# koszullab/chromosight

Measured on AMD Instinct MI355X. Metric: Mpixels/s normxcorr2 (17x17 loops kernel), higher is better.
Workload: dtype f32

## Files before the change

chromosight_amd/csrc/cs_corr_mfma.hip:

```cpp
#include "cs_device.h"
#include <algorithm>
#include <cstdlib>
#include <cstring>
#include <mutex>
#include <utility>
#include <vector>

#include "cs_launch.h"

namespace cs {

typedef _Float16 h8 __attribute__((ext_vector_type(8)));

__device__ __forceinline__ float cand_range_guard(float r, float s2, float unscale, const KernelStats<float>& K);
typedef _Float16 h4 __attribute__((ext_vector_type(4)));
typedef float f4 __attribute__((ext_vector_type(4)));
typedef float f4u __attribute__((ext_vector_type(4), aligned(4)));
typedef double d2u __attribute__((ext_vector_type(2), aligned(8)));

constexpr int MF_T = 64;
constexpr int MF_R = 80;
constexpr int MF_PLANE = MF_R * MF_R * 2;
constexpr int MF_WSET = 17 * 2 * 1024;
constexpr int MF_SCR_PITCH = 40;
constexpr int MF_SCR_PLANE = 16 * MF_SCR_PITCH * 2;
constexpr int MF_SMEM = 3 * MF_PLANE + MF_WSET + 64;
constexpr int MF_PER_THREAD = (MF_R * MF_R) / 256;

static_assert(5 * MF_SCR_PLANE * 4 <= MF_WSET, "scratch aliases the weight region");

#ifdef CS_MF_DEBUG
#define MFD_DBG(bit) (A.dbg & (bit))
#else
#define MFD_DBG(bit) (false)
#endif

#ifdef CS_MF_PROFILE
__device__ unsigned long long cs_mf_prof[16];
#define MF_STAMP(k)                                                        \
    do {                                                                   \
        const unsigned long long now_ = __builtin_readcyclecounter();      \
        if (tid == 0) MF_PROF_ADD(k, now_ - tprev_);                       \
        tprev_ = now_;                                                     \
    } while (0)
#define MF_PROF_ADD(k, v) atomicAdd(&cs_mf_prof[k], (unsigned long long)(v))
#else
#define MF_STAMP(k)
#endif

__device__ __forceinline__ f4 mfma16(const h8& a, const h8& b, const f4& c)
{
    return __builtin_amdgcn_mfma_f32_16x16x32_f16(a, b, c, 0, 0, 0);
}

template <bool MASKED>
__global__ __launch_bounds__(256, 2) void corr_mfma_kernel(const CorrArgs<float> A, const MfmaWeights E)
{
    extern __shared__ __attribute__((aligned(16))) char smem[];
    _Float16* xh = reinterpret_cast<_Float16*>(smem);
    _Float16* xl = reinterpret_cast<_Float16*>(smem + MF_PLANE);
    _Float16* xm = reinterpret_cast<_Float16*>(smem + 2 * MF_PLANE);
    char* wreg = smem + 3 * MF_PLANE;
    unsigned* red = reinterpret_cast<unsigned*>(wreg + MF_WSET);

    const int tid = threadIdx.x;
    const int lane = tid & 63, wv = tid >> 6;
    const int n = lane & 15, g = lane >> 4;

    const int by = blockIdx.x / A.tiles_x;
    const int bx = blockIdx.x - by * A.tiles_x;
    const int I0 = A.row_begin + by * MF_T;
    if (I0 >= A.row_end) return;
    const bool band_out = A.out.layout == 1;
    const int J0 = band_out ? I0 + A.out_lo + bx * MF_T : bx * MF_T;
    if (J0 >= A.ns || J0 + MF_T <= 0) return;
    if (J0 + MF_T - 1 - I0 < A.out_lo || J0 - (I0 + MF_T - 1) > A.out_hi) return;
#ifdef CS_MF_PROFILE
    unsigned long long tprev_ = __builtin_readcyclecounter();
    if (tid == 0) atomicAdd(&cs_mf_prof[15], 1ull);
#endif
    const int km = A.km, kn = A.kn;
    const int P0 = I0 - (km - 1) / 2, Q0 = J0 - (kn - 1) / 2;
    const int p_lo = A.row_begin - (km - 1) / 2, p_hi = A.row_end + (km - 1) - (km - 1) / 2;

    float xv[MF_PER_THREAD];
    unsigned miss_bits = 0, ok_bits = 0;
    long long offs[MF_PER_THREAD];
#pragma unroll
    for (int k = 0; k < MF_PER_THREAD; ++k) {
        const int idx = tid + 256 * k;
        const int r = idx / MF_R, c = idx - r * MF_R;
        const int p = P0 + r, q = Q0 + c;
        const bool inside = (p >= 0) & (p < A.ms) & (q >= 0) & (q < A.ns) & (p >= p_lo) & (p < p_hi);
        const long long off = inside ? mat_offset(A.sig, p, q) : -1;
        if (off >= 0) ok_bits |= 1u << k;
        offs[k] = off >= 0 ? off : 0;
    }
    if (A.sig_is_f64) {
        const double* src = reinterpret_cast<const double*>(A.sig.ptr);
#pragma unroll
        for (int k = 0; k < MF_PER_THREAD; ++k) xv[k] = (float)src[offs[k]];
    } else {
        const float* src = reinterpret_cast<const float*>(A.sig.ptr);
#pragma unroll
        for (int k = 0; k < MF_PER_THREAD; ++k) xv[k] = src[offs[k]];
    }
    if constexpr (MASKED) {
        unsigned char fr[MF_PER_THREAD], fc[MF_PER_THREAD];
        if (A.mask_mode == 1) {
#pragma unroll
            for (int k = 0; k < MF_PER_THREAD; ++k) {
                const int idx = tid + 256 * k;
                const int r = idx / MF_R, c = idx - r * MF_R;
                fr[k] = A.miss_row[min(max(P0 + r, 0), A.ms - 1)];
                fc[k] = A.miss_col[min(max(Q0 + c, 0), A.ns - 1)];
            }
        } else {
            const unsigned char* mp = reinterpret_cast<const unsigned char*>(A.mask.ptr);
#pragma unroll
            for (int k = 0; k < MF_PER_THREAD; ++k) {
                fr[k] = mp[offs[k]];
                fc[k] = 0;
            }
        }
#pragma unroll
        for (int k = 0; k < MF_PER_THREAD; ++k) {
            const int idx = tid + 256 * k;
            const int r = idx / MF_R, c = idx - r * MF_R;
            const int p = P0 + r, q = Q0 + c;
            const bool stored = (ok_bits >> k) & 1u;
            const bool needed = (p >= p_lo) & (p < p_hi);
            if (needed && missing_from_flags(A, p, q, fr[k] != 0, fc[k] != 0, fr[k] != 0, stored)) miss_bits |= 1u << k;
        }
    }
    float amax = 0.0f;
#pragma unroll
    for (int k = 0; k < MF_PER_THREAD; ++k) {
        const float x = (((ok_bits & ~miss_bits) >> k) & 1u) ? xv[k] : 0.0f;
        xv[k] = x;
        amax = fmaxf(amax, fabsf(x));
    }
    MF_STAMP(0);
    if (tid == 0) *red = 0u;
    __syncthreads();
#pragma unroll
    for (int off = 32; off >= 1; off >>= 1) amax = fmaxf(amax, __shfl_xor(amax, off));
    if (lane == 0) atomicMax(red, __float_as_uint(amax));
    __syncthreads();
    int ex = 0;
    {
        const int e = (int)((*red >> 23) & 0xffu);
        if (e != 0 && e != 255) ex = 6 - (e - 127);
        ex = max(-100, min(100, ex));
    }
    const float scale = __uint_as_float((unsigned)(ex + 127) << 23);
    const float unscale = __uint_as_float((unsigned)(127 - ex) << 23);
#pragma unroll
    for (int k = 0; k < MF_PER_THREAD; ++k) {
        const int idx = tid + 256 * k;
        const float xs = xv[k] * scale;
        const _Float16 h = (_Float16)xs;
        xh[idx] = h;
        xl[idx] = (_Float16)(xs - (float)h);
        if constexpr (MASKED) xm[idx] = (miss_bits >> k) & 1u ? (_Float16)1.0f : (_Float16)0.0f;
    }
    __syncthreads();

    MF_STAMP(1);
    h8 ones_b, ones_a;
#pragma unroll
    for (int e = 0; e < 8; ++e) {
        const int t = 8 * g + e - n;
        ones_b[e] = (t >= 0 && t < kn) ? (_Float16)1.0f : (_Float16)0.0f;
        ones_a[e] = (t >= 0 && t < km) ? (_Float16)1.0f : (_Float16)0.0f;
    }
    const f4 zero4 = {0.0f, 0.0f, 0.0f, 0.0f};
    const int wr0 = 16 * wv;

    f4 S1[4], S2[4], NM[4];
    char* scr = wreg + wv * (5 * MF_SCR_PLANE);
#pragma unroll
    for (int c = 0; c < 4; ++c) {
#pragma unroll
        for (int rb = 0; rb < 2; ++rb) {
            const int off = (wr0 + 16 * rb + n) * MF_R + 16 * c + 8 * g;
            const h8 ah = *reinterpret_cast<const h8*>(xh + off);
            const h8 al = *reinterpret_cast<const h8*>(xl + off);
            f4 h1 = mfma16(ah, ones_b, zero4);
            h1 = mfma16(al, ones_b, h1);
            h8 qh, ql;
#pragma unroll
            for (int e = 0; e < 8; ++e) {
                const float x = (float)ah[e] + (float)al[e];
                const float q = x * x * 0.03125f;
                qh[e] = (_Float16)q;
                ql[e] = (_Float16)(q - (float)qh[e]);
            }
            f4 h2 = mfma16(qh, ones_b, zero4);
            h2 = mfma16(ql, ones_b, h2);
            h4 t1h, t1l, t2h, t2l;
#pragma unroll
            for (int v = 0; v < 4; ++v) {
                t1h[v] = (_Float16)h1[v];
                t1l[v] = (_Float16)(h1[v] - (float)t1h[v]);
                t2h[v] = (_Float16)h2[v];
                t2l[v] = (_Float16)(h2[v] - (float)t2h[v]);
            }
            const int so = (n * MF_SCR_PITCH + 16 * rb + 4 * g) * 2;
            *reinterpret_cast<h4*>(scr + 0 * MF_SCR_PLANE + so) = t1h;
            *reinterpret_cast<h4*>(scr + 1 * MF_SCR_PLANE + so) = t1l;
            *reinterpret_cast<h4*>(scr + 2 * MF_SCR_PLANE + so) = t2h;
            *reinterpret_cast<h4*>(scr + 3 * MF_SCR_PLANE + so) = t2l;
            if constexpr (MASKED) {
                const h8 am = *reinterpret_cast<const h8*>(xm + off);
                const f4 hm = mfma16(am, ones_b, zero4);
                h4 tm;
#pragma unroll
                for (int v = 0; v < 4; ++v) tm[v] = (_Float16)hm[v];
                *reinterpret_cast<h4*>(scr + 4 * MF_SCR_PLANE + so) = tm;
            }
        }
        __syncthreads();
        {
            const int ro = (n * MF_SCR_PITCH + 8 * g) * 2;
            const h8 b1h = *reinterpret_cast<const h8*>(scr + 0 * MF_SCR_PLANE + ro);
            const h8 b1l = *reinterpret_cast<const h8*>(scr + 1 * MF_SCR_PLANE + ro);
            const h8 b2h = *reinterpret_cast<const h8*>(scr + 2 * MF_SCR_PLANE + ro);
            const h8 b2l = *reinterpret_cast<const h8*>(scr + 3 * MF_SCR_PLANE + ro);
            S1[c] = mfma16(ones_a, b1h, zero4);
            S1[c] = mfma16(ones_a, b1l, S1[c]);
            S2[c] = mfma16(ones_a, b2h, zero4);
            S2[c] = mfma16(ones_a, b2l, S2[c]);
            NM[c] = zero4;
            if constexpr (MASKED) {
                const h8 bm = *reinterpret_cast<const h8*>(scr + 4 * MF_SCR_PLANE + ro);
                NM[c] = mfma16(ones_a, bm, zero4);
            }
        }
        __syncthreads();
    }

    MF_STAMP(2);
    auto load_set = [&](int set) {
        const uint4* src = E.frag + (size_t)set * km * 128;
        uint4* dst = reinterpret_cast<uint4*>(wreg);
        for (int idx = tid; idx < km * 128; idx += 256) dst[idx] = src[idx];
    };
    f4 accM[4], accC[4], KA[4], KB[4];
#pragma unroll
    for (int c = 0; c < 4; ++c) accM[c] = accC[c] = KA[c] = KB[c] = zero4;

    load_set(0);
    __syncthreads();
    MF_STAMP(3);
    for (int s = 0; s < km; ++s) {
        const h8 bh = reinterpret_cast<const h8*>(wreg)[(2 * s + 0) * 64 + lane];
        const h8 bl = reinterpret_cast<const h8*>(wreg)[(2 * s + 1) * 64 + lane];
#pragma unroll
        for (int c = 0; c < 4; ++c) {
            const int off = (wr0 + s + n) * MF_R + 16 * c + 8 * g;
            const h8 ah = *reinterpret_cast<const h8*>(xh + off);
            const h8 al = *reinterpret_cast<const h8*>(xl + off);
            accM[c] = mfma16(ah, bh, accM[c]);
            accC[c] = mfma16(ah, bl, accC[c]);
            accC[c] = mfma16(al, bh, accC[c]);
        }
    }
    MF_STAMP(4);
    if constexpr (MASKED) {
        for (int set = 1; set <= 2; ++set) {
            __syncthreads();
            load_set(set);
            __syncthreads();
            for (int s = 0; s < km; ++s) {
                const h8 bh = reinterpret_cast<const h8*>(wreg)[(2 * s + 0) * 64 + lane];
                const h8 bl = reinterpret_cast<const h8*>(wreg)[(2 * s + 1) * 64 + lane];
#pragma unroll
                for (int c = 0; c < 4; ++c) {
                    const int off = (wr0 + s + n) * MF_R + 16 * c + 8 * g;
                    const h8 am = *reinterpret_cast<const h8*>(xm + off);
                    if (set == 1) {
                        KA[c] = mfma16(am, bh, KA[c]);
                        KA[c] = mfma16(am, bl, KA[c]);
                    } else {
                        KB[c] = mfma16(am, bh, KB[c]);
                        KB[c] = mfma16(am, bl, KB[c]);
                    }
                }
            }
        }
    }

    MF_STAMP(5);
    const float u_cs = unscale * E.unscale[0];
    const float u_s2 = 32.0f * unscale;
#pragma unroll
    for (int c = 0; c < 4; ++c) {
        const int j = J0 + 16 * c + n;
#pragma unroll
        for (int v = 0; v < 4; ++v) {
            const int i = I0 + wr0 + 4 * g + v;
            if (i >= A.row_end || j < 0 || j >= A.ns) continue;
            const int d = j - i;
            if (d < A.out_lo || d > A.out_hi) continue;
            const float cs = (accM[c][v] + accC[c][v]) * u_cs;
            const float s1 = S1[c][v] * unscale;
            const float s2 = (S2[c][v] * u_s2) * unscale;
            float r, nobs = A.ks.n;
            if (pixel_forced_zero(A, i, j)) {
                r = 0.0f;
            } else if (A.xcorr_only) {
                r = (fabsf(cs) < A.ks.thr) ? 0.0f : cs;
            } else if constexpr (MASKED) {
                const float nm = NM[c][v];
                const float ka = KA[c][v] * E.unscale[1], kb = KB[c][v] * E.unscale[2];
                r = cand_range_guard(pearson_masked_lean(cs, s1, s2, nm, ka, kb, A.ks), s2, unscale, A.ks);
                nobs = A.ks.n - nm;
            } else {
                r = cand_range_guard(pearson_nomask_lean(cs, s1, s2, A.ks), s2, unscale, A.ks);
            }
            store_pixel(A, i, j, r, nobs);
        }
    }
    MF_STAMP(6);
}

#ifdef CS_MF_PROFILE
extern "C" int cs_debug_mfma_profile(unsigned long long* out)
{
    hipError_t e = hipMemcpyFromSymbol(out, HIP_SYMBOL(cs_mf_prof), sizeof(cs_mf_prof));
    if (e != hipSuccess) return (int)e;
    unsigned long long zero[16] = {0};
    return (int)hipMemcpyToSymbol(HIP_SYMBOL(cs_mf_prof), zero, sizeof(zero));
}
#endif

struct MfmaFixArgs {
    int fix_on, fix_hi_w, fix_hi_d0;
    const float* fix_lo;
    const float* fix_hi;
    const float* fix_rows;
    const float* fix_cols;
    int fix_top, fix_bot0, fix_width, fix_xband, fix_xlo, fix_side;
    const float* rim;
    int max_dist;
};

struct MfmaDenseArgs {
    const float* sig;
    void* out;
    int out_is_f64;
    long long ld_in, ld_out, row0_in, row0_out;
    int ms, ns, km, kn;
    int row_begin, row_end;
    int full, sym_upper;
    int xcorr_only;
    int tiles_x, n_tiles;
    int by_cut;
    const uint4* frag;
    float w_unscale;
    float wa_unscale, wb_unscale;
    int xcd_order;
    int dbg;
    KernelStats<float> ks;
    int band_in, lo_in, bw_in;
    int pad_in;
    int cnt_in;
    int band_out, lo_out;
    int out_lo, out_hi;
    float* nobs;
    const float* w;
    const uint8_t* miss_col;
    const float* rowtab;
    const float* coltab;
    int fix_on, fix_hi_w, fix_hi_d0, fix_top, fix_bot0, fix_any_side;
    int rim_in_kernel;
    MfmaFixArgs fx;
};

constexpr int MFD_ROWS_PER_THREAD = 14;
constexpr int MFD_WL = 4 * MF_PLANE;
constexpr int MFD_SCR = MFD_WL + 18 * 1024;
constexpr int MFD_RED = MFD_SCR + 4 * 2 * MF_SCR_PLANE;
constexpr int MFD_SMEM = MFD_RED + 64;
constexpr int MFD_COL = MFD_RED + 64;
constexpr int MFD_CFL = MFD_COL + 2 * 3 * 64 * 4;
constexpr int MFD_CFB = MFD_CFL + 2 * 16;
constexpr int MFD_SMEM_REG = MFD_CFB + 2 * 128;
static_assert(MFD_SMEM_REG <= 80 * 1024, "two workgroups per CU");
#ifdef CS_MF_PROFILE
constexpr int MFD_PROF = MFD_SMEM_REG;
constexpr int MFD_LAUNCH_EXTRA = 128;
#else
constexpr int MFD_LAUNCH_EXTRA = 0;
#endif

__device__ __forceinline__ unsigned pack_h2(_Float16 a, _Float16 b)
{
    typedef _Float16 h2 __attribute__((ext_vector_type(2)));
    h2 v;
    v[0] = a;
    v[1] = b;
    return __builtin_bit_cast(unsigned, v);
}

__device__ __forceinline__ float sub_f16_lo(float x, unsigned h)
{
    float r;
    asm("v_fma_mix_f32 %0, -%1, 1.0, %2 op_sel_hi:[1,0,0]" : "=v"(r) : "v"(h), "v"(x));
    return r;
}

__device__ __forceinline__ float sub_f16_hi(float x, unsigned h)
{
    float r;
    asm("v_fma_mix_f32 %0, -%1, 1.0, %2 op_sel:[1,0,0] op_sel_hi:[1,0,0]" : "=v"(r) : "v"(h), "v"(x));
    return r;
}

__device__ __forceinline__ void lds_barrier()
{
    __builtin_amdgcn_fence(__ATOMIC_RELEASE, "workgroup", "local");
    __builtin_amdgcn_s_waitcnt(0xc07f);
    __builtin_amdgcn_s_barrier();
    __builtin_amdgcn_fence(__ATOMIC_ACQUIRE, "workgroup", "local");
}

__device__ __forceinline__ float wave_max_nonneg(float v)
{
#define CS_DPP_MAX(ctrl, rmask)                                                                                  \
    v = fmaxf(v, __builtin_bit_cast(float, __builtin_amdgcn_update_dpp(0, __builtin_bit_cast(int, v), ctrl, rmask, 0xf, true)))
    CS_DPP_MAX(0x111, 0xf);
    CS_DPP_MAX(0x112, 0xf);
    CS_DPP_MAX(0x114, 0xf);
    CS_DPP_MAX(0x118, 0xf);
    CS_DPP_MAX(0x142, 0xa);
    CS_DPP_MAX(0x143, 0xc);
#undef CS_DPP_MAX
    return v;
}

__device__ __forceinline__ void wave_lds_sync()
{
    __builtin_amdgcn_fence(__ATOMIC_RELEASE, "wavefront");
    __builtin_amdgcn_wave_barrier();
    __builtin_amdgcn_fence(__ATOMIC_ACQUIRE, "wavefront");
}

__device__ __forceinline__ float cand_range_guard(float r, float s2, float unscale, const KernelStats<float>& K)
{
    if (K.cand_cmin > 0.0f) r = ((int)(s2 > 0.0f) & (int)(s2 < K.n * (unscale * unscale) * 0.0625f)) ? 2.0f : r;
    return r;
}

__device__ __attribute__((noinline)) float masked_coefficient_rare(float cs, float s1, float s2, float nm, float ka, float kb,
                                                                   const KernelStats<float>& K)
{
    return pearson_masked_f32(cs, s1, s2, nm, ka, kb, K);
}

__device__ __forceinline__ float masked_coefficient(float cs, float s1, float s2, float nm, float ka, float kb,
                                                    const KernelStats<float>& K)
{
    bool rare;
    float r = pearson_masked_core(cs, s1, s2, nm, ka, kb, K, rare);
    if (rare) r = masked_coefficient_rare(cs, s1, s2, nm, ka, kb, K);
    return r;
}

typedef const __attribute__((address_space(4))) MfmaFixArgs* FixArgsPtr;

__device__ __forceinline__ FixArgsPtr fix_args()
{
    unsigned long long kv = (unsigned long long)__builtin_amdgcn_kernarg_segment_ptr();
    asm volatile("" : "+s"(kv));
    return (FixArgsPtr)(kv + offsetof(MfmaDenseArgs, fx));
}

typedef const __attribute__((address_space(4))) KernelStats<float>* StatsPtr;

__device__ __forceinline__ StatsPtr stats_args()
{
    unsigned long long kv = (unsigned long long)__builtin_amdgcn_kernarg_segment_ptr();
    asm volatile("" : "+s"(kv));
    return (StatsPtr)(kv + offsetof(MfmaDenseArgs, ks));
}
// ... 459 lines not shown
```

chromosight_amd/csrc/cs_corr_mfma_body.inc:

```

    extern __shared__ __attribute__((aligned(16))) char smem[];
    char* const pl_xh = smem;
    char* const pl_xl = smem + MF_PLANE;
    char* const pl_qh = smem + 2 * MF_PLANE;
    char* const pl_ql = smem + 3 * MF_PLANE;
    float* const raw = reinterpret_cast<float*>(smem + 2 * MF_PLANE);
    const int tid = threadIdx.x;
    const int lane = tid & 63, wv = tid >> 6;
    const int n = lane & 15, g = lane >> 4;
    char* const scr = smem + MFD_SCR + wv * (2 * MF_SCR_PLANE);
    unsigned* const red = reinterpret_cast<unsigned*>(smem + MFD_RED);
    const int km = A.km, kn = A.kn;
    const int kh = (km - 1) / 2, kw = (kn - 1) / 2;
#ifdef CS_MF_PROFILE
#undef MF_PROF_ADD
#define MF_PROF_ADD(k, v) (prof_lds[k] += (unsigned long long)(v))
    unsigned long long* const prof_lds = reinterpret_cast<unsigned long long*>(smem + MFD_PROF);
    unsigned long long tprev_ = 0;
    if (tid == 0)
        for (int k = 0; k < 16; ++k) prof_lds[k] = 0;
    auto prof_flush = [&]() {
        if (tid == 0)
            for (int k = 0; k < 16; ++k)
                if (prof_lds[k]) atomicAdd(&cs_mf_prof[k], prof_lds[k]);
    };
#endif

    h8 ones_b, ones_p;
#pragma unroll
    for (int e = 0; e < 8; ++e) {
        const int t = 8 * g + e - n;
        ones_b[e] = (t >= 0 && t < kn) ? (_Float16)1.0f : (_Float16)0.0f;
        const int rho = (e < 4 ? 4 * g + e : 16 + 4 * g + (e - 4)) - n;
        ones_p[e] = (rho >= 0 && rho < km) ? (_Float16)1.0f : (_Float16)0.0f;
    }
    const f4 zero4 = {0.0f, 0.0f, 0.0f, 0.0f};
    const int wr0 = 16 * wv;
    const int c2 = tid % 40, rg = tid / 40;
    const int c2_ = c2, rg_ = rg;
    const bool stager = tid < 240;
    const int p_min = max(0, A.row_begin - kh), p_max = min(A.ms, A.row_end + (km - 1) - kh) - 1;
    int pad_row0 = 0x7fffffff;
    if constexpr (REG && VEC4) pad_row0 = A.pad_in ? max(p_min, (int)A.row0_in + 1) : 0x7fffffff;
    float cnt_max = 0.0f;
    const float* cnt_wt = nullptr;
    const float* cnt_rlaw = nullptr;
    int cnt_n = 1, cnt_nd = 1;
    if constexpr (REG && VEC4) {
        if (A.cnt_in) {
            const CountsHdrPtr H = counts_header(A.sig);
            cnt_max = (float)H->max_val;
            cnt_wt = H->weight32;
            cnt_rlaw = H->rlaw32;
            cnt_n = H->n;
            cnt_nd = H->n_diags;
        }
    }

    auto tile_origin = [&](int tile, int& I0, int& J0) {
        if constexpr (LIST) tile = tile_list[tile];
        int by = tile / A.tiles_x;
        int bx = tile - by * A.tiles_x;
        if constexpr (REG) {
            if (by >= A.by_cut) {
                int t = tile - A.by_cut * A.tiles_x;
                by = A.by_cut;
                for (;;) {
                    const int left = A.ns - (A.row_begin + by * MF_T + A.out_lo);
                    const int v = min(A.tiles_x, left <= 0 ? 0 : (left + MF_T - 1) / MF_T);
                    if (t < v) break;
                    t -= v;
                    ++by;
                }
                bx = t;
            }
        }
        I0 = A.row_begin + by * MF_T;
        if constexpr (!REG) {
            const int skew = A.xcd_order >> 1;
            if (skew) {
                bx += (by * skew) % A.tiles_x;
                bx -= bx >= A.tiles_x ? A.tiles_x : 0;
            }
        }
        J0 = bx * MF_T;
        if (REG && A.band_out) J0 += I0 + A.out_lo;
    };
    const int wv_u = __builtin_amdgcn_readfirstlane(wv);
    auto fetch_args = [&]() {
        if constexpr (REG) return TABLE ? args_at(table_entry) : args_here();
        else return &A;
    };
    constexpr int kPiecesPerRow = VEC4 ? MF_R / 4 : MF_R;
    constexpr int kTransfers = VEC4 ? 25 : 100;
    auto fetch = [&](int tile, int slot) {
        const auto FA = fetch_args();
        int I0, J0;
        tile_origin(tile, I0, J0);
        const int P0 = I0 - kh, Q0 = J0 - kw;
        const bool pad_tile = REG && VEC4 && P0 >= pad_row0 && P0 + MF_R - 1 <= p_max;
        int lane_f = lane;
        if constexpr (REG) asm volatile("" : "+v"(lane_f));
        const int e0 = 64 * wv_u + lane_f;
        int r = e0 / kPiecesPerRow, c = e0 - r * kPiecesPerRow;
        if (REG && !MFD_DBG(16384)) {
            if (wv_u < 3) {
                const float* src = FA->coltab + (size_t)wv_u * FA->ns + min(max(J0 + lane_f, 0), FA->ns - 1);
                __builtin_amdgcn_global_load_lds(src, (__attribute__((address_space(3))) void*)(
                    (__attribute__((address_space(3))) char*)(smem) + MFD_COL + (slot * 3 + wv_u) * 256), 4, 0, 0);
            } else {
                const long long base = (long long)(uintptr_t)FA->miss_col;
                const long long first = ((base + Q0) >> 2) << 2;
                long long addr = first + 4 * min(lane_f, 23);
                addr = min(max(addr, (base >> 2) << 2), ((base + FA->ns - 1) >> 2) << 2);
                if (lane_f < 24)
                    __builtin_amdgcn_global_load_lds(reinterpret_cast<const unsigned*>((uintptr_t)addr),
                                                     (__attribute__((address_space(3))) void*)(
                                                         (__attribute__((address_space(3))) char*)(smem) + MFD_CFB + slot * 128), 4, 0, 0);
            }
        }
        if constexpr (REG && VEC4) {
            if (FA->cnt_in) {
                const float* wt = cnt_wt;
                const float* rlaw = cnt_rlaw;
                const int hn = cnt_n, hd = cnt_nd;
#pragma unroll 1
                for (int x = wv_u; x < 5; x += 4) {
                    const int e = 64 * x + lane_f;
                    const bool is_w = e < 160;
                    const int idx = e < 80 ? P0 + e : e < 160 ? Q0 + (e - 80) : Q0 - P0 - (MF_R - 1) + (e - 160);
                    const float* src = (is_w ? wt : rlaw) + min(max(idx, is_w ? 0 : -1), is_w ? hn - 1 : hd);
                    __builtin_amdgcn_global_load_lds(src, (__attribute__((address_space(3))) void*)(
                                                              (__attribute__((address_space(3))) char*)(smem) + MFD_SCR + 256 * x), 4, 0, 0);
                }
            }
        }
        const __attribute__((address_space(3))) char* dst =
            (const __attribute__((address_space(3))) char*)(raw) + (VEC4 ? 1024 : 256) * wv_u;
        if constexpr (!REG && VEC4) {
            if (P0 >= p_min && P0 + MF_R - 1 <= p_max && Q0 >= 0 && Q0 + MF_R <= FA->ns) {
                const float* src = FA->sig + ((long long)P0 + r - FA->row0_in) * FA->ld_in + Q0 + 4 * c;
                const long long step_r = 12 * FA->ld_in + 64, wrap = FA->ld_in - 80;
#pragma unroll 1
                for (int i = wv_u; i < kTransfers; i += 4) {
                    __builtin_amdgcn_global_load_lds(src, (__attribute__((address_space(3))) void*)dst, 16, 0, 0);
                    dst += 4096;
                    c += 16;
                    src += step_r;
                    if (c >= kPiecesPerRow) {
                        c -= kPiecesPerRow;
                        src += wrap;
                    }
                }
                return;
            }
        }
        if constexpr (REG && VEC4) {
            if (FA->band_in && P0 >= p_min && P0 + MF_R - 1 <= p_max && Q0 - (P0 + MF_R - 1) - FA->lo_in >= 0 &&
                Q0 + MF_R - 1 - P0 - FA->lo_in <= FA->bw_in - 1) {
                const float* src = FA->sig + ((long long)P0 - FA->row0_in) * FA->ld_in + (Q0 - P0 - FA->lo_in) + (long long)r * (FA->ld_in - 1) + 4 * c;
                const long long step_r = 12 * (FA->ld_in - 1) + 64, wrap = (FA->ld_in - 1) - 80;
#pragma unroll 1
                for (int i = wv_u; i < kTransfers; i += 4) {
                    __builtin_amdgcn_global_load_lds(src, (__attribute__((address_space(3))) void*)dst, 16, 0, 0);
                    dst += 4096;
                    c += 16;
                    src += step_r;
                    if (c >= kPiecesPerRow) {
                        c -= kPiecesPerRow;
                        src += wrap;
                    }
// ... 396 lines not shown
                           (!A.sym_upper || J0 - (I0 + MF_T - 1) + (A.full ? kn - km : 0) >= 0);
        const int i = I0 + wr0 + n;
        const long long o_idx = ((long long)i - A.row0_out) * A.ld_out + (J0 + 4 * g);
        f4 rv[4];
        bool lean = !A.xcorr_only && !MFD_DBG(32) && !(MFD_NOMASK_KS.cand_cmin > 0.0f);
        if (lean) {
            const KernelStats<float>& KS = MFD_NOMASK_KS;
            const float inv_u = __uint_as_float((254u << 23) - __float_as_uint(unscale));
            const float t1 = KS.thr_n * inv_u;
            const float t2 = (t1 * inv_u) * 0.03125f;
            const float td = (KS.den2_min * inv_u) * inv_u;
            const float top = (fmaxf(KS.kvar, 1.0f) * 4294967296.0f) * (unscale * unscale);
            auto normal_or_0 = [](float x) { return x == 0.0f || (x >= 1.17549435e-38f && x <= 3.40282347e38f); };
            lean = normal_or_0(t1) && normal_or_0(t2) && normal_or_0(td) && td > 0.0f && top <= 3.40282347e38f;
            if (lean) {
                const float n32 = 32.0f * KS.n, wu = A.w_unscale;
                bool normal = true;
#pragma unroll
                for (int c = 0; c < 4; ++c) {
#pragma unroll
                    for (int v = 0; v < 4; ++v) {
                        const float s1 = S1[c][v], s2 = S2[c][v], cw = acc[c][v] * wu;
                        const float den2 = fmaf(s2, n32, -s1 * s1) * KS.kvar;
                        float r = cw * __builtin_amdgcn_rsqf(den2);
                        r = (den2 >= td) ? r : 0.0f;
                        rv[c][v] = __builtin_amdgcn_fmed3f(r, -1.0f, 1.0f);
                        normal &= (int)(fabsf(s1) >= t1) & (int)(s2 >= t2) & (int)(fabsf(fmaf(KS.kmean, s1, cw)) >= t1);
                    }
                }
                lean = !__builtin_amdgcn_ballot_w64(!normal);
            }
        }
        if (!lean)
#pragma unroll
        for (int c = 0; c < 4; ++c) {
#pragma unroll
            for (int v = 0; v < 4; ++v) {
                const float cs = acc[c][v] * u_cs;
                const float s1 = S1[c][v] * unscale;
                const float s2 = (S2[c][v] * u_s2) * unscale;
                rv[c][v] = A.xcorr_only ? (fabsf(cs) < A.ks.thr ? 0.0f : cs)
                                        : MFD_DBG(32) ? cs + s1 + s2
                                                       : cand_range_guard(pearson_nomask_lean(cs, s1, s2, MFD_NOMASK_KS), s2, unscale, MFD_NOMASK_KS);
            }
        }
        if MFD_DBG(1) {
            if (rv[0][0] == 123.456f) reinterpret_cast<float*>(A.out)[o_idx] = rv[1][1] + rv[2][2] + rv[3][3];
        } else if (plain && VEC4) {
            float* tb = reinterpret_cast<float*>(scr);
            const long long r_idx = ((long long)(I0 + wr0 + (lane >> 3)) - A.row0_out) * A.ld_out + J0 + 4 * (lane & 7);
#pragma unroll
            for (int half = 0; half < 2; ++half) {
                wave_lds_sync();
                *reinterpret_cast<f4*>(tb + n * 36 + 4 * g) = rv[2 * half];
                *reinterpret_cast<f4*>(tb + n * 36 + 16 + 4 * g) = rv[2 * half + 1];
                wave_lds_sync();
                const f4 lo = *reinterpret_cast<const f4*>(tb + (lane >> 3) * 36 + 4 * (lane & 7));
                const f4 hi = *reinterpret_cast<const f4*>(tb + ((lane >> 3) + 8) * 36 + 4 * (lane & 7));
                if (A.out_is_f64) {
                    typedef double d2 __attribute__((ext_vector_type(2)));
                    double* od = reinterpret_cast<double*>(A.out) + r_idx + 32 * half;
                    d2 a, b;
                    a[0] = lo[0]; a[1] = lo[1]; b[0] = lo[2]; b[1] = lo[3];
                    *reinterpret_cast<d2*>(od) = a;
                    *reinterpret_cast<d2*>(od + 2) = b;
                    a[0] = hi[0]; a[1] = hi[1]; b[0] = hi[2]; b[1] = hi[3];
                    *reinterpret_cast<d2*>(od + 8 * A.ld_out) = a;
                    *reinterpret_cast<d2*>(od + 8 * A.ld_out + 2) = b;
                } else {
                    float* of = reinterpret_cast<float*>(A.out) + r_idx + 32 * half;
                    *reinterpret_cast<f4*>(of) = lo;
                    *reinterpret_cast<f4*>(of + 8 * A.ld_out) = hi;
                }
            }
        } else {
#pragma unroll
            for (int c = 0; c < 4; ++c) {
#pragma unroll
                for (int v = 0; v < 4; ++v) {
                    const int j = J0 + 16 * c + 4 * g + v;
                    bool z = false;
                    if (!A.full) z = (i < kh) | (i > A.ms - km + kh) | (j < kw) | (j > A.ns - kn + kw);
                    if (A.sym_upper) z = z | ((j - i) + (A.full ? (kn - km) : 0) < 0);
                    if (i < A.row_end && j < A.ns) {
                        const float val = z ? 0.0f : rv[c][v];
                        if (A.out_is_f64) reinterpret_cast<double*>(A.out)[o_idx + 16 * c + v] = (double)val;
                        else reinterpret_cast<float*>(A.out)[o_idx + 16 * c + v] = val;
                    }
                }
            }
        }
        }
    };

    f4 p_acc[4], p_S1[4], p_S2[4], p_hdr = zero4;
    int p_I0 = 0, p_J0 = 0, p_slot = 0, slot = 0;
    float p_unscale = 0.0f;
    bool pending = false;
#pragma unroll
    for (int c = 0; c < 4; ++c) p_acc[c] = p_S1[c] = p_S2[c] = zero4;

    int tile, tile_end, tile_step;
    if constexpr (TABLE) {
        tile = table_tile;
        tile_end = table_tile_end;
        tile_step = table_tile_step;
    } else if ((A.xcd_order & 1) && gridDim.x % 8 == 0) {
        const int x = blockIdx.x & 7, per = (A.n_tiles + 7) / 8;
        tile = x * per + (blockIdx.x >> 3);
        tile_end = min(A.n_tiles, (x + 1) * per);
        tile_step = gridDim.x >> 3;
    } else {
        tile = blockIdx.x;
        tile_end = A.n_tiles;
        tile_step = gridDim.x;
    }
    if MFD_DBG(2048) return;
    if (tile < tile_end) fetch(tile, 0);

    constexpr int kHeads = RSYM ? 1 : 17;
    h8 wh[kHeads];
    {
        const h8* frag = reinterpret_cast<const h8*>(A.frag);
        h8 z;
#pragma unroll
        for (int e = 0; e < 8; ++e) z[e] = (_Float16)0.0f;
        if constexpr (!RSYM) {
#pragma unroll
            for (int s = 0; s < kHeads; ++s) {
                const int sc = min(s, km - 1);
                const h8 a = frag[(2 * sc + 0) * 64 + lane];
                wh[s] = s < km ? a : z;
            }
        } else {
            wh[0] = z;
        }
        constexpr int kSlots = RSYM ? 18 : 17;
        h8 tails[5];
#pragma unroll
        for (int k = 0; k < 5; ++k) {
            const int idx = min(tid + 256 * k, kSlots * 64 - 1);
            const int slot = idx >> 6;
            const int row = RSYM ? (slot < 9 ? slot : slot - 9) : slot, part = RSYM ? (slot < 9 ? 1 : 0) : 1;
            tails[k] = frag[(2 * min(row, km - 1) + part) * 64 + (idx & 63)];
        }
#pragma unroll
        for (int k = 0; k < 5; ++k) {
            const int idx = tid + 256 * k;
            const int slot = idx >> 6;
            const int row = RSYM ? (slot < 9 ? slot : slot - 9) : slot;
            if (idx < kSlots * 64) reinterpret_cast<h8*>(smem + MFD_WL)[idx] = row < km ? tails[k] : z;
        }
    }
    for (;; tile += tile_step) {
        const bool have = REG ? tile < tile_end : true;
        if constexpr (REG) {
            if (!have && !pending) break;
        } else {
            if (tile >= tile_end) break;
        }
        int I0 = 0, J0 = 0;
        if (have) tile_origin(tile, I0, J0);
        const int P0 = I0 - kh, Q0 = J0 - kw;
        bool inside = P0 >= p_min && P0 + MF_R - 1 <= p_max && Q0 >= 0 && Q0 + MF_R <= A.ns;
        if (REG && A.band_in) inside = inside && Q0 - (P0 + MF_R - 1) - A.lo_in >= 0 && Q0 + MF_R - 1 - P0 - A.lo_in <= A.bw_in - 1;
        if (REG && VEC4) inside = inside || (P0 >= pad_row0 && P0 + MF_R - 1 <= p_max);
        if (REG && MFD_DBG(512)) inside = true;
        if MFD_DBG(1024) {
            if (!have) break;
            continue;
        }
        float unscale = 0.0f;
#ifdef CS_MF_PROFILE
        tprev_ = __builtin_readcyclecounter();
        if (tid == 0 && have) prof_lds[15] += 1ull;
#endif
        if (have) {

            bool cnt_tile = false;
            if constexpr (REG && VEC4) cnt_tile = A.cnt_in != 0;

            __builtin_amdgcn_s_waitcnt(0x0f70);
            lds_barrier();
            float xa[MFD_ROWS_PER_THREAD], xb[MFD_ROWS_PER_THREAD];
            float amax = 0.0f;
            if (inside) {
#pragma unroll
                for (int k = 0; k < MFD_ROWS_PER_THREAD; ++k) {
                    const int r = rg + 6 * k;
                    float2 v = make_float2(0.0f, 0.0f);
                    if (stager && r < MF_R) v = *reinterpret_cast<const float2*>(raw + r * MF_R + 2 * c2);
                    xa[k] = v.x;
                    xb[k] = v.y;
                    amax = fmaxf(amax, fmaxf(fabsf(v.x), fabsf(v.y)));
                }
            } else {
                int c2 = c2_, rg = rg_;
                if constexpr (REG) asm volatile("" : "+v"(c2), "+v"(rg));
#pragma unroll
                for (int k = 0; k < MFD_ROWS_PER_THREAD; ++k) {
                    const int r = rg + 6 * k;
                    float a = 0.0f, b = 0.0f;
                    if (REG && VEC4) {
                        if (stager && r < MF_R) {
                            const int p = P0 + r, q = Q0 + 2 * c2, cs = (2 * c2) & ~3;
                            const int w = A.band_in ? A.bw_in : A.ns;
                            const int off = A.band_in ? p + A.lo_in : 0;
                            const int idx_s = Q0 + cs - off;
                            const int idx_c = min(max(idx_s, 0), w - 4);
                            const int oa = (2 * c2 - cs) + (idx_s - idx_c), ob = oa + 1;
                            const int idx_a = q - off;
                            const bool rok = (p >= p_min) & (p <= p_max);
                            const bool oka = rok & (q >= 0) & (q < A.ns) & (idx_a >= 0) & (idx_a < w) & (oa >= 0) & (oa < 4);
                            const bool okb = rok & (q + 1 >= 0) & (q + 1 < A.ns) & (idx_a + 1 >= 0) & (idx_a + 1 < w) & (ob >= 0) & (ob < 4);
                            const float* piece = raw + r * MF_R + cs;
                            a = oka ? piece[min(max(oa, 0), 3)] : 0.0f;
                            b = okb ? piece[min(max(ob, 0), 3)] : 0.0f;
                        }
                    } else if (stager && r < MF_R) {
                        const float2 v = *reinterpret_cast<const float2*>(raw + r * MF_R + 2 * c2);
                        const int p = P0 + r, q = Q0 + 2 * c2;
                        const bool rok = (p >= p_min) & (p <= p_max);
                        bool oka = rok & (q >= 0) & (q < A.ns), okb = rok & (q + 1 >= 0) & (q + 1 < A.ns);
                        if (REG && A.band_in) {
                            const int dd = q - p - A.lo_in;
                            oka &= (dd >= 0) & (dd < A.bw_in);
                            okb &= (dd + 1 >= 0) & (dd + 1 < A.bw_in);
                        }
                        a = oka ? v.x : 0.0f;
                        b = okb ? v.y : 0.0f;
                    }
                    xa[k] = a;
                    xb[k] = b;
                    amax = fmaxf(amax, fmaxf(fabsf(a), fabsf(b)));
                }
            }
            if (cnt_tile) {
                const float* cwin = reinterpret_cast<const float*>(smem + MFD_SCR);
                int c2 = c2_, rg = rg_;
                asm volatile("" : "+v"(c2), "+v"(rg));
                typedef float f2 __attribute__((ext_vector_type(2)));
                const f2 cw = *reinterpret_cast<const f2*>(cwin + 80 + 2 * c2);
                const float max_f = cnt_max > 0.0f ? cnt_max : __uint_as_float(0x7f800000u);
                float thin_min = __uint_as_float(0x7f800000u);
                float fa[MFD_ROWS_PER_THREAD], fb[MFD_ROWS_PER_THREAD];
                amax = 0.0f;
                const float* wrow = cwin + rg;
                const float* rld = cwin + 160 + (MF_R - 1) + 2 * c2 - rg - 6 * (MFD_ROWS_PER_THREAD - 1);
#pragma unroll
                for (int k = 0; k < MFD_ROWS_PER_THREAD; ++k) {
                    const float rwk = wrow[6 * k];
                    f2 rl;
                    rl[0] = rld[6 * (MFD_ROWS_PER_THREAD - 1 - k)];
                    rl[1] = rld[6 * (MFD_ROWS_PER_THREAD - 1 - k) + 1];
                    f2 x;
                    x[0] = xa[k];
                    x[1] = xb[k];
                    f2 o = ((x * f2{rwk, rwk}) * cw) * rl;
                    const f2 t = o - f2{max_f, max_f};
                    thin_min = fminf(fminf(fabsf(t[0]), fabsf(t[1])), thin_min);
                    float a = fmaxf(o[0], 0.0f), b = fmaxf(o[1], 0.0f);
                    a = a >= max_f ? 1.0f : a;
                    b = b >= max_f ? 1.0f : b;
                    fa[k] = a;
                    fb[k] = b;
                    amax = fmaxf(amax, fmaxf(a, b));
                }
                bool thin_any = __builtin_amdgcn_ballot_w64(thin_min <= max_f * 2e-6f) != 0;
                if (thin_any && cnt_max > 0.0f) {
                    const CountsHdrPtr H = counts_header(A.sig);
                    const int hn = H->n, hd = H->n_diags;
                    const double* wt = H->weight + H->row0;
                    const double* law = H->law;
                    const double* rlaw = H->rlaw;
                    const double max_val = H->max_val;
                    amax = 0.0f;
#pragma unroll 1
                    for (int k = 0; k < MFD_ROWS_PER_THREAD; ++k) {
                        const int r = rg + 6 * k;
                        const int p = P0 + r, q = Q0 + 2 * c2, d = q - p;
                        const double rwk = wt[min(max(p, 0), hn - 1)];
                        float xk = 0.0f, yk = 0.0f;
                        if (stager && r < MF_R) {
                            if (inside) {
                                const float2 v = *reinterpret_cast<const float2*>(raw + r * MF_R + 2 * c2);
                                xk = v.x;
                                yk = v.y;
                            } else {
                                const int cs = (2 * c2) & ~3;
                                const int w = A.band_in ? A.bw_in : A.ns;
                                const int off = A.band_in ? p + A.lo_in : 0;
                                const int idx_s = Q0 + cs - off;
                                const int idx_c = min(max(idx_s, 0), w - 4);
                                const int oa = (2 * c2 - cs) + (idx_s - idx_c), ob = oa + 1;
                                const int idx_a = q - off;
                                const bool rok = (p >= p_min) & (p <= p_max);
                                const bool oka = rok & (q >= 0) & (q < A.ns) & (idx_a >= 0) & (idx_a < w) & (oa >= 0) & (oa < 4);
                                const bool okb = rok & (q + 1 >= 0) & (q + 1 < A.ns) & (idx_a + 1 >= 0) & (idx_a + 1 < w) & (ob >= 0) & (ob < 4);
                                const float* piece = raw + r * MF_R + cs;
                                xk = oka ? piece[min(max(oa, 0), 3)] : 0.0f;
                                yk = okb ? piece[min(max(ob, 0), 3)] : 0.0f;
                            }
                        }
                        const int da = min(max(d, 0), hd - 1), db = min(max(d + 1, 0), hd - 1);
                        const float a = (float)stage_detrend_rcp(((double)xk * rwk) * wt[min(max(q, 0), hn - 1)], rlaw[da], max_val, law + da);
                        const float b = (float)stage_detrend_rcp(((double)yk * rwk) * wt[min(max(q + 1, 0), hn - 1)], rlaw[db], max_val, law + db);
#pragma unroll
                        for (int e = 0; e < MFD_ROWS_PER_THREAD; ++e) {
                            fa[e] = e == k ? a : fa[e];
                            fb[e] = e == k ? b : fb[e];
                        }
                        amax = fmaxf(amax, fmaxf(fabsf(a), fabsf(b)));
                    }
                }
#pragma unroll
                for (int k = 0; k < MFD_ROWS_PER_THREAD; ++k) {
                    xa[k] = fa[k];
                    xb[k] = fb[k];
                }
            }
            amax = wave_max_nonneg(amax);
            if (lane == 63) red[wv] = __float_as_uint(amax);
            if constexpr (REG) {
                if (wv < 2) {
                    const int q = Q0 + tid;
                    const long long start = (long long)(uintptr_t)A.miss_col + Q0;
                    const int skew = (int)(start - ((start >> 2) << 2));
                    const uint8_t fb = reinterpret_cast<const uint8_t*>(smem + MFD_CFB)[slot * 128 + skew + min(tid, 79)];
                    const bool flagged = tid < 80 && q >= 0 && q < A.ns && fb;
                    const unsigned long long m = __builtin_amdgcn_ballot_w64(flagged);
                    unsigned* cfm = reinterpret_cast<unsigned*>(smem + MFD_CFL) + slot * 4;
                    if (lane == 0) {
                        cfm[2 * wv] = (unsigned)m;
                        if (wv == 0) cfm[1] = (unsigned)(m >> 32);
                    }
                }
            }
            MF_STAMP(0);
            lds_barrier();
            int ex = 0;
            {
                const uint4 m4 = *reinterpret_cast<const uint4*>(red);
                const unsigned mx = max(max(m4.x, m4.y), max(m4.z, m4.w));
                const int e = (int)((mx >> 23) & 0xffu);
                if (e != 0 && e != 255) ex = 6 - (e - 127);
                ex = max(-100, min(100, ex));
            }
            const float scale = __uint_as_float((unsigned)(ex + 127) << 23);
            const float qscale = __uint_as_float((unsigned)(ex + 127 - 5) << 23);
            unscale = __uint_as_float((unsigned)(127 - ex) << 23);
            typedef __fp16 hv2 __attribute__((ext_vector_type(2)));
#pragma unroll
            for (int k = 0; k < MFD_ROWS_PER_THREAD; ++k) {
                const int r = rg + 6 * k;
                if (stager && r < MF_R && !MFD_DBG(16)) {
                    const float a = xa[k] * scale, b = xb[k] * scale;
                    const hv2 hh = __builtin_amdgcn_cvt_pkrtz(a, b);
                    const float qa = (xa[k] * qscale) * a, qb = (xb[k] * qscale) * b;
                    const hv2 qh = __builtin_amdgcn_cvt_pkrtz(qa, qb);
                    hv2 tt, qt;
                    if constexpr (!REG) {
                        const unsigned hu = __builtin_bit_cast(unsigned, hh), qu = __builtin_bit_cast(unsigned, qh);
                        tt = __builtin_amdgcn_cvt_pkrtz(sub_f16_lo(a, hu), sub_f16_hi(b, hu));
                        qt = __builtin_amdgcn_cvt_pkrtz(sub_f16_lo(qa, qu), sub_f16_hi(qb, qu));
                    } else {
                        tt = __builtin_amdgcn_cvt_pkrtz(a - (float)hh[0], b - (float)hh[1]);
                        qt = __builtin_amdgcn_cvt_pkrtz(qa - (float)qh[0], qb - (float)qh[1]);
                    }
                    const int o = (r * MF_R + 2 * c2) * 2;
                    *reinterpret_cast<hv2*>(pl_xh + o) = hh;
                    *reinterpret_cast<hv2*>(pl_xl + o) = tt;
                    *reinterpret_cast<hv2*>(pl_qh + o) = qh;
                    *reinterpret_cast<hv2*>(pl_ql + o) = qt;
                }
            }
            MF_STAMP(1);
        } else if (REG) {
            __builtin_amdgcn_s_waitcnt(0x0f70);
            lds_barrier();
        }
        if (pending) emit(p_I0, p_J0, p_unscale, p_acc, p_S1, p_S2, p_hdr, p_slot);
        if (!have) break;
        MF_STAMP(6);
        lds_barrier();

        f4 S1[4], S2[4];
#pragma unroll
        for (int c = 0; c < 4; ++c) S1[c] = S2[c] = zero4;
        if (!MFD_DBG(4) && !A.xcorr_only) {
            auto hfrag = [&](int t, h8 (&f)[4]) {
                const int c = t >> 1;
                const char* ph = (t & 1) ? pl_qh : pl_xh;
                const char* pt = (t & 1) ? pl_ql : pl_xl;
#pragma unroll
                for (int rb = 0; rb < 2; ++rb) {
                    const int off = ((wr0 + 16 * rb + n) * MF_R + 16 * c + 8 * g) * 2;
                    f[2 * rb] = *reinterpret_cast<const h8*>(ph + off);
                    f[2 * rb + 1] = *reinterpret_cast<const h8*>(pt + off);
                }
            };
            h8 cur[4];
            hfrag(0, cur);
#pragma unroll
            for (int t = 0; t < 8; ++t) {
                h8 nxt[4];
                if (t + 1 < 8) hfrag(t + 1, nxt);
                h8 bh, bl;
                typedef unsigned u4 __attribute__((ext_vector_type(4)));
                u4 bhw, blw;
#pragma unroll
                for (int rb = 0; rb < 2; ++rb) {
                    f4 h = mfma16(cur[2 * rb], ones_b, zero4);
                    h = mfma16(cur[2 * rb + 1], ones_b, h);
                    if constexpr (!REG) {
#pragma unroll
                        for (int pr = 0; pr < 2; ++pr) {
                            const unsigned hp = pack_h2((_Float16)h[2 * pr], (_Float16)h[2 * pr + 1]);
                            bhw[2 * rb + pr] = hp;
                            blw[2 * rb + pr] = pack_h2((_Float16)sub_f16_lo(h[2 * pr], hp), (_Float16)sub_f16_hi(h[2 * pr + 1], hp));
                        }
                    } else {
#pragma unroll
                        for (int v = 0; v < 4; ++v) {
                            const _Float16 hh = (_Float16)h[v];
                            bh[4 * rb + v] = hh;
                            bl[4 * rb + v] = (_Float16)(h[v] - (float)hh);
                        }
                    }
                }
                if constexpr (!REG) {
                    bh = __builtin_bit_cast(h8, bhw);
                    bl = __builtin_bit_cast(h8, blw);
                }
                f4 sacc = mfma16(bh, ones_p, zero4);
                sacc = mfma16(bl, ones_p, sacc);
                if (t & 1) S2[t >> 1] = sacc;
                else S1[t >> 1] = sacc;
                if (t + 1 < 8) {
#pragma unroll
                    for (int q = 0; q < 4; ++q) cur[q] = nxt[q];
                }
            }
        }
        MF_STAMP(2);
        lds_barrier();
        if (tile + tile_step < tile_end && !MFD_DBG(2)) fetch(tile + tile_step, slot ^ 1);

        MF_STAMP(3);
        f4 acc[4];
#pragma unroll
        for (int c = 0; c < 4; ++c) acc[c] = zero4;
        h8 ah[4], al[4], bl;
        const int fo = ((wr0 + n) * MF_R + 8 * g) * 2;
#pragma unroll
        for (int c = 0; c < 4; ++c) {
            ah[c] = *reinterpret_cast<const h8*>(pl_xh + fo + 32 * c);
            al[c] = *reinterpret_cast<const h8*>(pl_xl + fo + 32 * c);
        }
        h8 bh;
        bl = reinterpret_cast<const h8*>(smem + MFD_WL)[lane];
        if constexpr (RSYM) bh = reinterpret_cast<const h8*>(smem + MFD_WL)[9 * 64 + lane];
        else bh = wh[0];
        if (!MFD_DBG(8))
#pragma unroll
        for (int s = 0; s < 17; ++s) {
            h8 nh[4], nl[4], nb, nbh;
            if (s + 1 < 17) {
#pragma unroll
                for (int c = 0; c < 4; ++c) {
                    nh[c] = *reinterpret_cast<const h8*>(pl_xh + fo + (s + 1) * MF_R * 2 + 32 * c);
                    nl[c] = *reinterpret_cast<const h8*>(pl_xl + fo + (s + 1) * MF_R * 2 + 32 * c);
                }
                const int sn = RSYM && s + 1 > 8 ? 16 - (s + 1) : s + 1;
                nb = reinterpret_cast<const h8*>(smem + MFD_WL)[sn * 64 + lane];
                if constexpr (RSYM) nbh = reinterpret_cast<const h8*>(smem + MFD_WL)[(9 + sn) * 64 + lane];
                else nbh = wh[s + 1];
            }
            __builtin_amdgcn_sched_barrier(0);
#pragma unroll
            for (int c = 0; c < 4; ++c) acc[c] = mfma16(bh, ah[c], acc[c]);
#pragma unroll
            for (int c = 0; c < 4; ++c) acc[c] = mfma16(bl, ah[c], acc[c]);
#pragma unroll
            for (int c = 0; c < 4; ++c) acc[c] = mfma16(bh, al[c], acc[c]);
            __builtin_amdgcn_sched_barrier(0);
            if (s + 1 < 17) {
#pragma unroll
                for (int c = 0; c < 4; ++c) {
                    ah[c] = nh[c];
                    al[c] = nl[c];
                }
                bl = nb;
                bh = nbh;
            }
        }
        MF_STAMP(4);
#pragma unroll
        for (int c = 0; c < 4; ++c) {
            p_acc[c] = acc[c];
            p_S1[c] = S1[c];
            p_S2[c] = S2[c];
        }
        p_I0 = I0;
        p_J0 = J0;
        p_unscale = unscale;
        p_slot = slot;
        if constexpr (REG) p_hdr = *reinterpret_cast<const f4*>(A.rowtab + 4 * (size_t)min(I0 + wr0 + n, A.ms - 1));
        slot ^= 1;
        pending = true;
    }
    if constexpr (!REG) {
        if (pending) emit(p_I0, p_J0, p_unscale, p_acc, p_S1, p_S2, p_hdr, p_slot);
    }
#ifdef CS_MF_PROFILE
    prof_flush();
#undef MF_PROF_ADD
#define MF_PROF_ADD(k, v) atomicAdd(&cs_mf_prof[k], (unsigned long long)(v))
#endif
```

Before: 218,900.

## Interleave box-sum MFMAs with cross-correlation MFMA loop in non-REG path

```diff
diff --git a/chromosight_amd/csrc/cs_corr_mfma.hip b/chromosight_amd/csrc/cs_corr_mfma.hip
--- a/chromosight_amd/csrc/cs_corr_mfma.hip
+++ b/chromosight_amd/csrc/cs_corr_mfma.hip
@@ -37,6 +37,8 @@
 
 #ifdef CS_MF_PROFILE
 __device__ unsigned long long cs_mf_prof[16];
+constexpr int MF_CLK_WG = 1024;
+__device__ unsigned long long cs_mf_clk[MF_CLK_WG][4];
 #define MF_STAMP(k)                                                        \
     do {                                                                   \
         const unsigned long long now_ = __builtin_readcyclecounter();      \
@@ -332,6 +334,18 @@
     if (e != hipSuccess) return (int)e;
     unsigned long long zero[16] = {0};
     return (int)hipMemcpyToSymbol(HIP_SYMBOL(cs_mf_prof), zero, sizeof(zero));
+}
+
+extern "C" int cs_debug_mfma_clock(unsigned long long* out, int* n_wg)
+{
+    *n_wg = MF_CLK_WG;
+    if (!out) return 0;
+    hipError_t e = hipMemcpyFromSymbol(out, HIP_SYMBOL(cs_mf_clk), sizeof(cs_mf_clk));
+    if (e != hipSuccess) return (int)e;
+    void* d = nullptr;
+    e = hipGetSymbolAddress(&d, HIP_SYMBOL(cs_mf_clk));
+    if (e != hipSuccess) return (int)e;
+    return (int)hipMemset(d, 0, sizeof(cs_mf_clk));
 }
 #endif
 
diff --git a/chromosight_amd/csrc/cs_corr_mfma_body.inc b/chromosight_amd/csrc/cs_corr_mfma_body.inc
--- a/chromosight_amd/csrc/cs_corr_mfma_body.inc
+++ b/chromosight_amd/csrc/cs_corr_mfma_body.inc
@@ -17,6 +17,7 @@
 #define MF_PROF_ADD(k, v) (prof_lds[k] += (unsigned long long)(v))
     unsigned long long* const prof_lds = reinterpret_cast<unsigned long long*>(smem + MFD_PROF);
     unsigned long long tprev_ = 0;
+    [[maybe_unused]] const unsigned long long clk_t0_ = __builtin_amdgcn_s_memtime();
     if (tid == 0)
         for (int k = 0; k < 16; ++k) prof_lds[k] = 0;
     auto prof_flush = [&]() {
@@ -719,6 +720,9 @@
             if (idx < kSlots * 64) reinterpret_cast<h8*>(smem + MFD_WL)[idx] = row < km ? tails[k] : z;
         }
     }
+#ifdef CS_MF_PROFILE
+    [[maybe_unused]] const unsigned long long clk_t1_ = __builtin_amdgcn_s_memtime(), clk_r1_ = __builtin_amdgcn_s_memrealtime();
+#endif
     for (;; tile += tile_step) {
         const bool have = REG ? tile < tile_end : true;
         if constexpr (REG) {
@@ -951,21 +955,123 @@
         MF_STAMP(6);
         lds_barrier();
 
-        f4 S1[4], S2[4];
-#pragma unroll
-        for (int c = 0; c < 4; ++c) S1[c] = S2[c] = zero4;
+        f4 S1[4], S2[4], acc[4];
+#pragma unroll
+        for (int c = 0; c < 4; ++c) S1[c] = S2[c] = acc[c] = zero4;
+        auto hfrag = [&](int t, h8 (&f)[4]) {
+            const int c = t >> 1;
+            const char* ph = (t & 1) ? pl_qh : pl_xh;
+            const char* pt = (t & 1) ? pl_ql : pl_xl;
+#pragma unroll
+            for (int rb = 0; rb < 2; ++rb) {
+                const int off = ((wr0 + 16 * rb + n) * MF_R + 16 * c + 8 * g) * 2;
+                f[2 * rb] = *reinterpret_cast<const h8*>(ph + off);
+                f[2 * rb + 1] = *reinterpret_cast<const h8*>(pt + off);
+            }
+        };
+        typedef unsigned u4 __attribute__((ext_vector_type(4)));
+        bool fused = false;
+        if constexpr (!REG) fused = !A.xcorr_only && !MFD_DBG(4 | 8);
+        if (fused) {
+            auto split = [&](const f4& h, int rb, u4& hw, u4& lw) {
+#pragma unroll
+                for (int pr = 0; pr < 2; ++pr) {
+                    const unsigned hp = pack_h2((_Float16)h[2 * pr], (_Float16)h[2 * pr + 1]);
+                    hw[2 * rb + pr] = hp;
+                    lw[2 * rb + pr] = pack_h2((_Float16)sub_f16_lo(h[2 * pr], hp), (_Float16)sub_f16_hi(h[2 * pr + 1], hp));
+                }
+            };
+            h8 ah[4], al[4], bl, bh, bf[4];
+            const int fo = ((wr0 + n) * MF_R + 8 * g) * 2;
+#pragma unroll
+            for (int c = 0; c < 4; ++c) {
+                ah[c] = *reinterpret_cast<const h8*>(pl_xh + fo + 32 * c);
+                al[c] = *reinterpret_cast<const h8*>(pl_xl + fo + 32 * c);
+            }
+            bl = reinterpret_cast<const h8*>(smem + MFD_WL)[lane];
+            if constexpr (RSYM) bh = reinterpret_cast<const h8*>(smem + MFD_WL)[9 * 64 + lane];
+            else bh = wh[0];
+            hfrag(0, bf);
+            f4 h0 = zero4, h1 = zero4, sv = zero4;
+            u4 bhw = {0u, 0u, 0u, 0u}, blw = {0u, 0u, 0u, 0u};
+#pragma unroll
+            for (int s = 0; s < 17; ++s) {
+                constexpr int kBox = 8;
+                h8 nh[4], nbh;
+                const int sn = RSYM && s + 1 > 8 ? 16 - (s + 1) : s + 1;
+                if (s + 1 < 17) {
+#pragma unroll
+                    for (int c = 0; c < 4; ++c) nh[c] = *reinterpret_cast<const h8*>(pl_xh + fo + (s + 1) * MF_R * 2 + 32 * c);
+                    if constexpr (RSYM) nbh = reinterpret_cast<const h8*>(smem + MFD_WL)[(9 + sn) * 64 + lane];
+                    else nbh = wh[s + 1];
+                }
+                __builtin_amdgcn_sched_barrier(0);
+                acc[0] = mfma16(bh, ah[0], acc[0]);
+                acc[1] = mfma16(bh, ah[1], acc[1]);
+                if (s >= 1 && s <= kBox) {
+                    sv = mfma16(__builtin_bit_cast(h8, blw), ones_p, sv);
+                    __builtin_amdgcn_sched_barrier(0);
+                }
+                acc[2] = mfma16(bh, ah[2], acc[2]);
+                acc[3] = mfma16(bh, ah[3], acc[3]);
+                if (s < kBox) {
+                    h0 = mfma16(bf[0], ones_b, zero4);
+                    h1 = mfma16(bf[2], ones_b, zero4);
+                }
+                __builtin_amdgcn_sched_barrier(0);
+                if (s >= 1 && s <= kBox) {
+                    if ((s - 1) & 1) S2[(s - 1) >> 1] = sv;
+                    else S1[(s - 1) >> 1] = sv;
+                }
+                acc[0] = mfma16(bl, ah[0], acc[0]);
+                acc[1] = mfma16(bl, ah[1], acc[1]);
+                if (s < kBox) {
+                    h0 = mfma16(bf[1], ones_b, h0);
+                    h1 = mfma16(bf[3], ones_b, h1);
+                    __builtin_amdgcn_sched_barrier(0);
+                    if (s + 1 < kBox) hfrag(s + 1, bf);
+                }
+                __builtin_amdgcn_sched_barrier(0);
+                acc[2] = mfma16(bl, ah[2], acc[2]);
+                acc[3] = mfma16(bl, ah[3], acc[3]);
+                __builtin_amdgcn_sched_barrier(0);
+                if (s + 1 < 17) bl = reinterpret_cast<const h8*>(smem + MFD_WL)[sn * 64 + lane];
+                __builtin_amdgcn_sched_barrier(0);
+                acc[0] = mfma16(bh, al[0], acc[0]);
+                __builtin_amdgcn_sched_barrier(0);
+                if (s < kBox) {
+                    split(h0, 0, bhw, blw);
+                    __builtin_amdgcn_sched_barrier(0);
+                }
+                acc[1] = mfma16(bh, al[1], acc[1]);
+                __builtin_amdgcn_sched_barrier(0);
+                if (s < kBox) {
+                    split(h1, 1, bhw, blw);
+                    __builtin_amdgcn_sched_barrier(0);
+                }
+                acc[2] = mfma16(bh, al[2], acc[2]);
+                acc[3] = mfma16(bh, al[3], acc[3]);
+                if (s < kBox) sv = mfma16(__builtin_bit_cast(h8, bhw), ones_p, zero4);
+                __builtin_amdgcn_sched_barrier(0);
+                if (s + 1 < 17) {
+#pragma unroll
+                    for (int c = 0; c < 4; ++c) {
+                        ah[c] = nh[c];
+                        al[c] = *reinterpret_cast<const h8*>(pl_xl + fo + (s + 1) * MF_R * 2 + 32 * c);
+                    }
+                    bh = nbh;
+                }
+                __builtin_amdgcn_sched_barrier(0);
+                if (s == kBox - 1) {
+                    MF_STAMP(2);
+                    lds_barrier();
+                    if (tile + tile_step < tile_end && !MFD_DBG(2)) fetch(tile + tile_step, slot ^ 1);
+                    MF_STAMP(3);
+                }
+            }
+            MF_STAMP(4);
+        } else {
         if (!MFD_DBG(4) && !A.xcorr_only) {
-            auto hfrag = [&](int t, h8 (&f)[4]) {
-                const int c = t >> 1;
-                const char* ph = (t & 1) ? pl_qh : pl_xh;
-                const char* pt = (t & 1) ? pl_ql : pl_xl;
-#pragma unroll
-                for (int rb = 0; rb < 2; ++rb) {
-                    const int off = ((wr0 + 16 * rb + n) * MF_R + 16 * c + 8 * g) * 2;
-                    f[2 * rb] = *reinterpret_cast<const h8*>(ph + off);
-                    f[2 * rb + 1] = *reinterpret_cast<const h8*>(pt + off);
-                }
-            };
             h8 cur[4];
             hfrag(0, cur);
 #pragma unroll
@@ -973,7 +1079,6 @@
                 h8 nxt[4];
                 if (t + 1 < 8) hfrag(t + 1, nxt);
                 h8 bh, bl;
-                typedef unsigned u4 __attribute__((ext_vector_type(4)));
                 u4 bhw, blw;
 #pragma unroll
                 for (int rb = 0; rb < 2; ++rb) {
@@ -1014,9 +1119,6 @@
         if (tile + tile_step < tile_end && !MFD_DBG(2)) fetch(tile + tile_step, slot ^ 1);
 
         MF_STAMP(3);
-        f4 acc[4];
-#pragma unroll
-        for (int c = 0; c < 4; ++c) acc[c] = zero4;
         h8 ah[4], al[4], bl;
         const int fo = ((wr0 + n) * MF_R + 8 * g) * 2;
 #pragma unroll
@@ -1062,6 +1164,7 @@
             }
         }
         MF_STAMP(4);
+        }
 #pragma unroll
         for (int c = 0; c < 4; ++c) {
             p_acc[c] = acc[c];
@@ -1076,10 +1179,22 @@
         slot ^= 1;
         pending = true;
     }
+#ifdef CS_MF_PROFILE
+    [[maybe_unused]] const unsigned long long clk_t2_ = __builtin_amdgcn_s_memtime(), clk_r2_ = __builtin_amdgcn_s_memrealtime();
+#endif
     if constexpr (!REG) {
         if (pending) emit(p_I0, p_J0, p_unscale, p_acc, p_S1, p_S2, p_hdr, p_slot);
     }
 #ifdef CS_MF_PROFILE
+    if constexpr (!REG && !TABLE) {
+        const unsigned long long clk_t3_ = __builtin_amdgcn_s_memtime();
+        if (tid == 0 && blockIdx.x < MF_CLK_WG) {
+            cs_mf_clk[blockIdx.x][0] = clk_t1_ - clk_t0_;
+            cs_mf_clk[blockIdx.x][1] = clk_t2_ - clk_t1_;
+            cs_mf_clk[blockIdx.x][2] = clk_t3_ - clk_t2_;
+            cs_mf_clk[blockIdx.x][3] = clk_r2_ - clk_r1_;
+        }
+    }
     prof_flush();
 #undef MF_PROF_ADD
 #define MF_PROF_ADD(k, v) atomicAdd(&cs_mf_prof[k], (unsigned long long)(v))
```

Result: faster. 222,000 (median of 6 runs) (+1.4%).
